# RajaeeKh/TriNerfLet

Measured on AMD Instinct MI355X. Metric: train rays/sec (whole node), higher is better.
Workload: dtype f16; 1 GPU; base: 3x32ch x 2048^2 planes, bior6.8 scale 32, hidden 64, 60000 rays/step/GPU, solid-sphere occupancy r=0.8 (re-imposed after each refresh), fp16 planes + fp16 MFMA MLP, fp32 masters, Adam+L1; GT colours = an analytic function of the ray direction (synthetic.target_colors), not a second seeded field's render; sample_budget_M=4769546, parallelism=ray-dp1

## Files before the change

### include/trinerflet_hip.h

```cpp
#ifndef TRINERFLET_HIP_H
#define TRINERFLET_HIP_H

#include <stdint.h>

#ifdef __cplusplus
extern "C" {
#endif

#define TNL_API __attribute__((visibility("default")))

TNL_API int tnl_abi_version(void);


TNL_API int tnl_near_far_from_aabb(const float *rays_o, const float *rays_d, const float *aabb,
                                   uint32_t N, float min_near, float *nears, float *fars,
                                   void *stream);

TNL_API int tnl_sph_from_ray(const float *rays_o, const float *rays_d, float radius, uint32_t N,
                             float *coords, void *stream);

TNL_API int tnl_morton3D(const int32_t *coords, uint32_t N, int32_t *indices, void *stream);

TNL_API int tnl_morton3D_invert(const int32_t *indices, uint32_t N, int32_t *coords, void *stream);

TNL_API int tnl_packbits(const float *grid, uint32_t N, float density_thresh, uint8_t *bitfield,
                         void *stream);
TNL_API int tnl_packbits_dev(const float *grid, uint32_t N, float density_thresh, const float *mean_density_dev,
                             uint8_t *bitfield, void *stream);

TNL_API int tnl_occupancy_bounds(const uint8_t *bitfield, uint32_t bytes_per_cascade, uint32_t cascades,
                                 int32_t *bounds, void *stream);
TNL_API int tnl_occupancy_row_extents(const uint8_t *bitfield, uint32_t bytes_per_cascade, uint32_t cascades, uint32_t H,
                                      float bound, uint32_t R, int32_t *ext, void *stream);

TNL_API int tnl_occupied_box(const uint8_t *bitfield, uint32_t bytes_per_cascade, uint32_t cascades, uint32_t H,
                             float bound, int32_t *bounds_scratch, float *box, void *stream);
TNL_API int tnl_clip_fars(const float *rays_o, const float *rays_d, const float *fars, const float *box, uint32_t N,
                          float *fars_out, void *stream);

TNL_API uint32_t tnl_march_rays_train_workspace(uint32_t N);
TNL_API uint32_t tnl_march_rays_train_workspace_rec(uint32_t N, uint32_t max_steps);

TNL_API int tnl_march_rays_train(const float *rays_o, const float *rays_d, const uint8_t *grid,
                                 float bound, float dt_gamma, uint32_t max_steps, uint32_t N,
                                 uint32_t C, uint32_t H, uint32_t M, const float *nears,
                                 const float *fars, float *xyzs, float *dirs, float *deltas,
                                 int32_t *rays, int32_t *counter, const float *noises,
                                 int32_t *workspace, uint32_t workspace_words, void *stream);
TNL_API int tnl_march_rays_train_binned(const float *rays_o, const float *rays_d, const uint8_t *grid,
                                 float bound, float dt_gamma, uint32_t max_steps, uint32_t N,
                                 uint32_t C, uint32_t H, uint32_t M, const float *nears,
                                 const float *fars, float *xyzs, float *dirs, float *deltas,
                                 int32_t *rays, int32_t *counter, const float *noises,
                                 int32_t *workspace, uint32_t workspace_words, uint32_t R, void *sort_workspace, void *stream);

TNL_API int tnl_march_count_form(int form);

TNL_API int tnl_march_emit_cap(int blocks);
TNL_API int tnl_plane_grad_fill_cap(int blocks);

TNL_API int tnl_composite_rays_train_forward(const float *sigmas, const float *rgbs,
                                             const float *deltas, const int32_t *rays, uint32_t M,
                                             uint32_t N, float T_thresh, float *weights_sum,
                                             float *depth, float *image, void *stream);

TNL_API int tnl_composite_rays_train_backward(const float *grad_weights_sum, const float *grad_image,
                                              const float *sigmas, const float *rgbs,
                                              const float *deltas, const int32_t *rays,
                                              const float *weights_sum, const float *image,
                                              uint32_t M, uint32_t N, float T_thresh,
                                              float *grad_sigmas, float *grad_rgbs, void *stream);

TNL_API int tnl_march_rays(uint32_t n_alive, uint32_t n_step, const int32_t *rays_alive,
                           const float *rays_t, const float *rays_o, const float *rays_d,
                           float bound, float dt_gamma, uint32_t max_steps, uint32_t C, uint32_t H,
                           const uint8_t *grid, const float *nears, const float *fars, float *xyzs,
                           float *dirs, float *deltas, const float *noises, void *stream);

TNL_API int tnl_composite_rays(uint32_t n_alive, uint32_t n_step, float T_thresh,
                               int32_t *rays_alive, float *rays_t, const float *sigmas,
                               const float *rgbs, const float *deltas, float *weights_sum,
                               float *depth, float *image, void *stream);

TNL_API int tnl_compact_rays(const int32_t *rays_alive, uint32_t n_alive, int32_t *rays_alive_out,
                             int32_t *n_out, int32_t *workspace, void *stream);

TNL_API int tnl_sh_encode_forward(const float *inputs, float *outputs, uint32_t B, uint32_t D,
                                  uint32_t C, float *dy_dx, void *stream);
TNL_API int tnl_sh_encode_backward(const float *grad, const float *inputs, uint32_t B, uint32_t D,
                                   uint32_t C, const float *dy_dx, float *grad_inputs, void *stream);


TNL_API int tnl_idwt_level_forward(const float *x, const float *yh, uint32_t S, uint32_t n,
                                   int wave, float *out, void *stream);

TNL_API int tnl_idwt_level_forward_half(const float *x, const float *yh, uint32_t S, uint32_t n,
                                        int wave, void *out_half, void *stream);

TNL_API int tnl_idwt_level_backward(const float *dout, uint32_t S, uint32_t n, int wave, float *dx,
                                    float *dyh, void *stream);

TNL_API int tnl_idwt_level_backward_adam(const float *dout, uint32_t S, uint32_t n, int wave, float *dx,
                                         float *p, float *m, float *v, float *ll_p, float *ll_m,
                                         float *ll_v, float step_size, float bias2_sqrt, float beta1,
                                         float beta2, float eps, float inv_scale,
                                         const float *inv_scale_dev, float l1_coef,
                                         const float *found_inf, float *abs_sum, void *stream);

TNL_API int tnl_planes_to_texel_major(const float *planes_cm, uint32_t C, uint32_t R, int half_out,
                                      void *planes_tm, void *stream);
TNL_API int tnl_planes_to_texel_major_win(const float *planes_cm, uint32_t C, uint32_t R, int half_out,
                                          void *planes_tm, const int32_t *roi, void *stream);
TNL_API int tnl_planes_half_to_texel_major(const void *planes_cm_half, uint32_t C, uint32_t R,
                                           void *planes_tm_half, void *stream);
TNL_API int tnl_planes_to_channel_major(const float *grad_tm, uint32_t C, uint32_t R, float *grad_cm,
                                        void *stream);

TNL_API int tnl_triplane_sample_forward(const void *planes_tm, int half_in, const float *xyz,
                                        float bound, uint32_t N, uint32_t C, uint32_t R, float *feats,
                                        void *stream);
TNL_API int tnl_triplane_sample_backward(const float *grad_feats, const float *xyz, float bound,
                                         uint32_t N, uint32_t C, uint32_t R, float *grad_tm,
                                         void *stream);

TNL_API int tnl_grid_sample_tm_forward(const void *planes_tm, int half_in, const float *grid, uint32_t N, uint32_t C,
                                       uint32_t CG, uint32_t R, float *feats, void *stream);
TNL_API int tnl_grid_sample_tm_backward(const void *planes_tm, int half_in, const float *grid,
                                        const float *grad_feats, uint32_t N, uint32_t C, uint32_t CG, uint32_t R,
                                        float *grad_tm, float *grad_grid, void *stream);

TNL_API uint32_t tnl_field_packed_bytes(uint32_t C, uint32_t Hd, uint32_t Hc);
TNL_API int tnl_field_pack(const float *W0, const float *W1, const float *W2, const float *W3,
                           const float *W4, uint32_t C, uint32_t Hd, uint32_t Hc, void *packed,
                           void *stream);
TNL_API uint64_t tnl_field_feats_save_bytes(uint32_t M, uint32_t C, uint32_t Hd);
TNL_API int tnl_field_forward(const void *planes_tm, int half_in, const float *xyz, const float *dirs,
                              float bound, uint32_t M, uint32_t C, uint32_t R, uint32_t Hd,
                              uint32_t Hc, const void *packed, float *sigma, float *rgb,
                              void *feats_save, const int32_t *m_actual, void *stream);
TNL_API uint64_t tnl_field_backward_workspace(uint32_t M, uint32_t C, uint32_t Hd, uint32_t Hc);
TNL_API int tnl_field_backward(const float *grad_sigma, const float *grad_rgb, const float *sigma,
                               const float *rgb, const void *feats_save, const float *xyz,
                               const float *dirs, float bound, uint32_t M, uint32_t C, uint32_t R,
                               uint32_t Hd, uint32_t Hc, const void *packed, float *grad_tm,
                               float *gradW, void *workspace, const int32_t *m_actual, void *dfeat_half,
                               void *stream);

TNL_API uint64_t tnl_plane_grad_binned_workspace(uint32_t M, uint32_t R);
TNL_API int tnl_plane_grad_binned(const void *dfeat_half, const float *xyz, float bound, uint32_t M,
                                  const int32_t *m_actual, uint32_t C, uint32_t R, float grad_scale,
                                  float *grad_out, int channel_major, int32_t *nonfinite_flag,
                                  void *workspace, void *stream);

TNL_API int tnl_plane_grad_sort_layout(uint32_t M, uint32_t R, int64_t *out);
TNL_API int tnl_plane_grad_sort(const float *xyz, float bound, uint32_t M, const int32_t *m_actual, uint32_t R,
                                void *workspace, void *stream);
TNL_API int tnl_plane_grad_sort_counted(const float *xyz, float bound, uint32_t M, const int32_t *m_actual,
                                        uint32_t R, void *workspace, void *stream);
TNL_API int tnl_plane_grad_reduce(const void *dfeat_half, const float *xyz, float bound, uint32_t M, uint32_t C,
                                  uint32_t R,
                                  float grad_scale, float *grad_out, int channel_major, int32_t *nonfinite_flag,
                                  const int32_t *roi, const void *workspace, void *stream);

TNL_API int tnl_idwt_level_forward_half_roi(const float *x, const float *yh, uint32_t S, uint32_t n, int wave,
                                            void *out_half, const int32_t *roi, void *stream);
TNL_API int tnl_planes_half_to_texel_major_roi(const void *planes_roi_half, uint32_t C, uint32_t R,
                                               void *planes_tm_half, const int32_t *roi, void *stream);
TNL_API int tnl_plane_grad_binned_roi(const void *dfeat_half, const float *xyz, float bound, uint32_t M,
                                      const int32_t *m_actual, uint32_t C, uint32_t R, float grad_scale,
                                      float *grad_out, int channel_major, int32_t *nonfinite_flag,
                                      const int32_t *roi, void *workspace, void *stream);
TNL_API int tnl_idwt_level_backward_roi(const float *dout_roi, uint32_t S, uint32_t n, int wave, float *dx,
                                        float *dyh, const int32_t *roi, void *stream);

TNL_API int tnl_adam_l1_step(float *p, float *grad, float *m, float *v, uint64_t n, float step_size,
                             float bias2_sqrt, float beta1, float beta2, float eps, float inv_scale,
                             const float *inv_scale_dev, float l1_coef, const float *found_inf,
                             float *abs_sum, int zero_grad, void *stream);
TNL_API int tnl_adam_l1_step_dev(float *p, float *grad, float *m, float *v, uint64_t n, float lr,
                                 const float *opt_step_dev, float beta1, float beta2, float eps, float inv_scale,
                                 const float *inv_scale_dev, float l1_coef, const float *found_inf,
                                 float *abs_sum, int zero_grad, void *stream);
TNL_API int tnl_adam_l1_step_sink(float *p, float *grad, float *m, float *v, uint64_t n, float lr,
                                  const float *opt_step_dev, float beta1, float beta2, float eps,
                                  const float *inv_scale_dev, float l1_coef, const float *l1_scaled_dev,
                                  const float *found_inf, void *stream);

TNL_API int tnl_mse_loss(const float *image, const float *weights_sum, const float *gt_rgb, float bg_color,
                         const float *bg_rays, uint32_t N, float inv_norm, const float *scale_dev, float *pred,
                         float *grad_pred, float *grad_weights_sum, float *mse_accum, void *stream);

TNL_API uint64_t tnl_abs_mean_workspace(void);
TNL_API int tnl_abs_mean_forward(const float *x, uint64_t n, void *workspace, float *out, void *stream);
TNL_API int tnl_abs_mean_backward(const float *x, uint64_t n, const float *grad_out, float *grad_x, void *stream);
TNL_API int tnl_nonfinite_check(const float *x, uint64_t n, float *found_inf, void *stream);

TNL_API int tnl_copy_probe(const void *src, void *dst, uint64_t bytes, void *stream);

TNL_API int tnl_step_prologue(const float *scale, float *inv_scale, float *abs_sum, int32_t *nonfinite, float *mse,
                              float *small_grad, uint32_t n, void *stream);
TNL_API int tnl_scaler_probe(const float *g0, uint32_t n0, const float *g1, uint32_t n1, const int32_t *nonfinite,
                             float *probe, float *found_inf, void *stream);
TNL_API int tnl_step_epilogue(const float *found_inf, float *opt_steps, float *scale, int32_t *growth_tracker,
                              float growth, float backoff, int32_t growth_interval, int32_t update_scale,
                              const float *abs_sum, float l1_coef, float *reg, void *stream);

TNL_API uint64_t tnl_permute_index(uint64_t g, uint64_t total, uint64_t key);
TNL_API int tnl_ray_batch(const float *poses, const float *intrinsics_host, uint32_t B, uint32_t H, uint32_t W,
                          const void *images, int channels, int images_u8, const int64_t *pix, uint64_t first,
                          uint64_t perm_total, uint64_t perm_key, uint32_t N, float bg_color,
                          const float *bg_rand, float *rays_o, float *rays_d, float *gt_rgb, int64_t *pix_out,
                          void *stream);

TNL_API int tnl_render_work(int units);

TNL_API int tnl_render_rays(const void *planes_tm, int half_in, uint32_t C, uint32_t R, uint32_t Hd, uint32_t Hc,
                            const void *packed, const float *rays_o, const float *rays_d, const float *nears,
                            const float *fars, uint32_t N, const uint8_t *grid, float bound, float dt_gamma,
                            uint32_t max_steps, uint32_t cascades, uint32_t H, float T_thresh, float density_scale,
                            const float *noises, int32_t *queue, float *weights_sum, float *depth, float *image,
                            void *stream);

TNL_API int tnl_infer_plan(int32_t *state, uint32_t N, uint32_t max_steps, uint32_t min_step, void *stream);
TNL_API int tnl_march_rays_dev(const int32_t *state, uint32_t N, const int32_t *rays_alive, const float *rays_t,
                               const float *rays_o, const float *rays_d, float bound, float dt_gamma,
                               uint32_t max_steps, uint32_t C, uint32_t H, const uint8_t *grid, const float *fars,
                               float *xyzs, float *dirs, float *deltas, const float *noises, float *t_scratch,
                               uint32_t rows_cap, void *stream);
TNL_API int tnl_composite_rays_dev(const int32_t *state, uint32_t N, float T_thresh, int32_t *rays_alive,
                                   float *rays_t, const float *sigmas, const float *rgbs, const float *deltas,
                                   float *weights_sum, float *depth, float *image, void *stream);
TNL_API int tnl_compact_rays_dev(int32_t *state, uint32_t N, const int32_t *rays_alive, int32_t *rays_alive_out,
                                 int32_t *workspace, void *stream);

TNL_API int tnl_idwt_level_forward_win(const float *x, const float *yh, uint32_t S, uint32_t n, int wave, float *out,
                                       const int32_t *win, void *stream);
TNL_API int tnl_idwt_level_backward_win(const float *dout, uint32_t S, uint32_t n, int wave, float *dx, float *dyh,
                                        const int32_t *win, int strided, int32_t *out_rect, void *stream);

TNL_API int tnl_idwt_set_walk_min_n(uint32_t walk_min_n);
TNL_API int tnl_idwt_get_walk_min_n(void);
TNL_API int tnl_idwt_level_forward_spans(const float *x, const float *yh, uint32_t S, uint32_t n, int wave, void *out,
                                         int half_out, const int32_t *win, int strided, const int32_t *spans,
                                         void *stream);
TNL_API int tnl_idwt_level_backward_spans(const float *dout, uint32_t S, uint32_t n, int wave, float *dx, float *dyh,
                                          const int32_t *win, int strided, int32_t *out_rect, const int32_t *spans,
                                          void *stream);
TNL_API int tnl_idwt_level_backward_live_adam(const float *dout, uint32_t S, uint32_t n, int wave, float *dx,
                                              const int32_t *win, int strided, const int32_t *live_rect,
                                              const int32_t *spans, float *p, float *m, float *v,
                                              const int32_t *band_table, uint32_t nb, const float *step_rec,
                                              float beta1, float beta2, float eps, float inv_scale,
                                              const float *inv_scale_dev, float l1_coef, const float *found_inf,
                                              float *abs_sum, void *stream);
TNL_API int tnl_planes_half_to_texel_major_spans(const void *planes_roi_half, uint32_t C, uint32_t R,
                                                 void *planes_tm_half, const int32_t *roi, const int32_t *spans,
                                                 void *stream);
TNL_API int tnl_idwt_set_tuning(int key, int value);
TNL_API int tnl_adam_l1_step_rect(float *p, float *grad, float *m, float *v, uint32_t S, uint32_t bands, uint32_t n,
                                  uint32_t spp, uint32_t s0, const int32_t *rect, float lr,
                                  const float *opt_step_dev, float beta1, float beta2, float eps, float inv_scale,
                                  const float *inv_scale_dev, float l1_coef, const float *found_inf,
                                  float *abs_sum, void *stream);
TNL_API int tnl_adam_record_step_dev(float *ring, int32_t slot, const float *lr_dev, const float *opt_step_dev, float beta1,
                                     float beta2, const float *found_inf, void *stream);
TNL_API int tnl_adam_l1_step_rec(float *p, float *grad, float *m, float *v, uint64_t n, const float *step_rec, float beta1,
                                 float beta2, float eps, const float *inv_scale_dev, float l1_coef,
                                 const float *found_inf, float *abs_sum, void *stream);
TNL_API int tnl_adam_l1_step_rect_rec(float *p, float *grad, float *m, float *v, uint32_t S, uint32_t bands, uint32_t n,
                                      uint32_t spp, uint32_t s0, const int32_t *rect, const float *step_rec, float beta1,
                                      float beta2, float eps, const float *inv_scale_dev, float l1_coef,
                                      const float *found_inf, float *abs_sum, void *stream);
TNL_API int tnl_adam_l1_step_live(float *p, float *grad, float *m, float *v, uint32_t S, uint32_t spp, uint32_t s0,
                                  uint32_t n_levels, const uint64_t *offsets, const uint32_t *sizes,
                                  const uint32_t *bands, const int32_t *live, const int32_t *grad_rect,
                                  const float *l1_coefs, float lr, const float *opt_step_dev, const float *step_rec,
                                  float beta1, float beta2, float eps, float inv_scale, const float *inv_scale_dev,
                                  const float *found_inf, float *abs_sum, void *stream);
TNL_API int tnl_adam_record_step(float *ring, int32_t slot, float lr, const float *opt_step_dev, float beta1,
                                 float beta2, const float *found_inf, void *stream);
TNL_API int tnl_adam_record_step_l1(float *ring, int32_t slot, float lr, const float *opt_step_dev, float beta1,
                                    float beta2, const float *found_inf, const float *l1_scaled_dev,
                                    const float *inv_scale_dev, void *stream);
TNL_API int tnl_adam_l1_catchup(float *p, float *m, float *v, uint32_t S, uint32_t bands, uint32_t n, uint32_t spp,
                                uint32_t s0, const int32_t *live, const float *ring, int32_t count, float beta1,
                                float beta2, float eps, float l1_coef, float *abs_sums, void *stream);
TNL_API int tnl_adam_l1_step_live_bands(float *p, float *grad, float *m, float *v, uint32_t S, uint32_t spp, uint32_t s0,
                                        uint32_t n_levels, const uint64_t *offsets, const uint32_t *sizes,
                                        const uint32_t *bands, const int32_t *live, const int32_t *grad_rect,
                                        const int32_t *const *band_tables, const uint32_t *band_quads,
                                        const float *l1_coefs, float lr, const float *opt_step_dev, const float *step_rec,
                                        float beta1, float beta2, float eps, float inv_scale, const float *inv_scale_dev,
// ... 11 lines not shown
```

### trinerflet_amd/csrc/field.hip

```cpp
#include <hip/hip_fp16.h>
#include <hip/hip_runtime.h>
#include <stdint.h>

#include "../../include/trinerflet_hip.h"
#include "field_device.h"

namespace {

#ifndef TNL_FWD_PREFETCH
#define TNL_FWD_PREFETCH 1
#endif
#ifndef TNL_FWD_LDSW
#define TNL_FWD_LDSW 0
#endif
#ifndef TNL_FWD_MINWAVES
#define TNL_FWD_MINWAVES 1
#endif
template <int C, int H, bool HALFP, bool DENSITY_ONLY, bool SAVE>
__global__ void __launch_bounds__(FWD_THREADS, TNL_FWD_MINWAVES)
k_field_fwd(const void* __restrict__ planes, const float* __restrict__ xyz, const float* __restrict__ dirs,
            float bound, uint32_t M, int R, const half8* __restrict__ packed, float* __restrict__ sigma,
            float* __restrict__ rgb, _Float16* __restrict__ feats_save, _Float16* __restrict__ geo_save,
            const int32_t* __restrict__ m_actual) {
  using G = FieldGeom<C, H>;
  if (m_actual != nullptr) M = min(M, (uint32_t)max(*m_actual, 0));
  if (M == 0) return;
  extern __shared__ __attribute__((aligned(16))) char smem[];
  half8* w = reinterpret_cast<half8*>(smem);
  constexpr int NFR = DENSITY_ONLY ? G::F2 : G::NF;
  constexpr int FT = FWD_THREADS;
  for (int i = threadIdx.x; i < NFR * 64; i += FT) w[i] = packed[i];
  __syncthreads();

  const int lane = threadIdx.x & 63, r = lane & 31, h = lane >> 5;
  const uint32_t waves = gridDim.x * (FT / 64);
  const uint32_t ntiles = (M + 31) / 32;
  const uint32_t tile0 = blockIdx.x * (FT / 64) + (threadIdx.x >> 6);
  float npx = 0.f, npy = 0.f, npz = 0.f, ndx = 0.f, ndy = 0.f, ndz = 0.f;
  auto fetch_pos = [&](uint32_t t) {
    const uint32_t i_ = t * 32 + r;
    const uint32_t il_ = i_ < M ? i_ : M - 1;
    npx = xyz[(size_t)il_ * 3]; npy = xyz[(size_t)il_ * 3 + 1]; npz = xyz[(size_t)il_ * 3 + 2];
    if (!DENSITY_ONLY) { ndx = dirs[(size_t)il_ * 3]; ndy = dirs[(size_t)il_ * 3 + 1]; ndz = dirs[(size_t)il_ * 3 + 2]; }
  };
  if (tile0 < ntiles) fetch_pos(tile0);
  for (uint32_t tile = tile0; tile < ntiles; tile += waves) {
#if TNL_FWD_LDSW
    asm volatile("" : "+s"(w));
#endif
    const uint32_t i = tile * 32 + r;
    const bool valid = i < M;
    const float px = npx, py = npy, pz = npz;
    const float cdx = ndx, cdy = ndy, cdz = ndz;
    if (tile + waves < ntiles) fetch_pos(tile + waves);
#ifndef TNL_FWD_PG128
#define TNL_FWD_PG128 1
#endif
    constexpr int PG = H > 64 ? TNL_FWD_PG128 : 3;
    const uint32_t il = valid ? i : M - 1;
    f32x16 acc0[G::OB];
#pragma unroll
    for (int ob = 0; ob < G::OB; ob++) acc0[ob] = zero16();
#pragma unroll
    for (int p0 = 0; p0 < 3; p0 += PG) {
      half8 fk[PG * (C / 16)];
#pragma unroll
      for (int p = p0; p < p0 + PG; p++) {
        TexelTap t;
        triplane_tap(px, py, pz, bound, R, p, t);
#pragma unroll
        for (int kk = 0; kk < C / 16; kk++) fk[(p - p0) * (C / 16) + kk] = gather_frag<C, HALFP>(planes, R, p, kk, h, t);
      }
      if (TNL_FWD_PREFETCH && H > 64) {
#pragma unroll
        for (int q = 0; q < PG * (C / 16); q++)
          if (SAVE) *reinterpret_cast<half8*>(feats_save + feat_slot<G::KS0>(il, p0 * (C / 16) + q, h)) = fk[q];
        with_weights<PG * (C / 16) * G::OB, G::OB>(
            [&](int i) { return w[(G::F0 + (i % G::OB) * G::KS0 + p0 * (C / 16) + i / G::OB) * 64 + lane]; },
            [&](int i, const half8& f) { acc0[i % G::OB] = MFMA32(f, fk[i / G::OB], acc0[i % G::OB]); });
      } else {
#pragma unroll
        for (int q = 0; q < PG * (C / 16); q++) {
          const int ks = p0 * (C / 16) + q;
          if (SAVE) *reinterpret_cast<half8*>(feats_save + feat_slot<G::KS0>(il, ks, h)) = fk[q];
#pragma unroll
          for (int ob = 0; ob < G::OB; ob++) acc0[ob] = MFMA32(w[(G::F0 + ob * G::KS0 + ks) * 64 + lane], fk[q], acc0[ob]);
        }
      }
      if (PG < 3) __builtin_amdgcn_sched_barrier(0);
    }
    const float dx = cdx, dy = cdy, dz = cdz;
    Chain<C, H> ch;
    chain_tail<C, H, DENSITY_ONLY, (TNL_FWD_PREFETCH && H > 64)>(w, w, lane, h, acc0, dx, dy, dz, ch);
    if (!DENSITY_ONLY && geo_save != nullptr && valid) {
      half8 g;
#pragma unroll
      for (int j = 0; j < 8; j++) g[j] = (_Float16)ch.o8[j];
      *reinterpret_cast<half8*>(geo_save + (size_t)i * 16 + 8 * h) = g;
    }
    if (valid && h == 0) {
      sigma[i] = expf(ch.o8[0]);
      if (!DENSITY_ONLY) {
        rgb[(size_t)i * 3 + 0] = 1.f / (1.f + expf(-ch.rgbl[0]));
        rgb[(size_t)i * 3 + 1] = 1.f / (1.f + expf(-ch.rgbl[1]));
        rgb[(size_t)i * 3 + 2] = 1.f / (1.f + expf(-ch.rgbl[2]));
      }
    }
    if (DENSITY_ONLY && rgb != nullptr && valid) {
#pragma unroll
      for (int g = 0; g < 8; g++) {
        const int row = acc_row(g, h);
        if (row >= 1) rgb[(size_t)i * 15 + row - 1] = ch.o8[g];
      }
    }
  }
}

template <int C, int H>
__global__ void k_field_pack(const float* __restrict__ W0, const float* __restrict__ W1, const float* __restrict__ W2,
                             const float* __restrict__ W3, const float* __restrict__ W4,
                             _Float16* __restrict__ packed) {
  using G = FieldGeom<C, H>;
  const int idx = blockIdx.x * blockDim.x + threadIdx.x;
  if (idx >= G::NTOT * 512) return;
  const int src = field_pack_source<C, H>(idx);
  float v = 0.f;
  if (src >= 0) {
    if (src < G::OFF1) v = W0[src - G::OFF0];
    else if (src < G::OFF2) v = W1[src - G::OFF1];
    else if (src < G::OFF3) v = W2[src - G::OFF2];
    else if (src < G::OFF4) v = W3[src - G::OFF3];
    else v = W4[src - G::OFF4];
  }
  packed[idx] = (_Float16)v;
}

template <int C, int H>
int launch_fwd(const void* planes, int half_in, const float* xyz, const float* dirs, float bound, uint32_t M,
               uint32_t R, const void* packed, float* sigma, float* rgb, void* feats_save, bool density_only,
               const int32_t* m_actual, hipStream_t st) {
  using G = FieldGeom<C, H>;
  const uint32_t ntiles = (M + 31) / 32;
  constexpr uint32_t WPB = FWD_THREADS / 64;
  uint32_t blocks = (ntiles + WPB - 1) / WPB;
  if (blocks > 2048) blocks = 2048;
  const half8* pk = reinterpret_cast<const half8*>(packed);
  _Float16* fs = reinterpret_cast<_Float16*>(feats_save);
  _Float16* gs = (split_backward<H>() && fs != nullptr) ? fs + (size_t)((M + 31) / 32 * 32) * G::F : nullptr;
#define TNL_LAUNCH(HP, DO, SV)                                                                                        \
  hipLaunchKernelGGL((k_field_fwd<C, H, HP, DO, SV>), dim3(blocks), dim3(FWD_THREADS), (DO ? G::F2 : G::NF) * 1024, st, \
                     planes, xyz, dirs, bound, M, (int)R, pk, sigma, rgb, fs, gs, m_actual)
#define TNL_LAUNCH_SV(HP, DO) do { if (fs != nullptr) TNL_LAUNCH(HP, DO, true); else TNL_LAUNCH(HP, DO, false); } while (0)
  if (density_only) {
    if (half_in) TNL_LAUNCH_SV(true, true); else TNL_LAUNCH_SV(false, true);
  } else {
    if (half_in) TNL_LAUNCH_SV(true, false); else TNL_LAUNCH_SV(false, false);
  }
#undef TNL_LAUNCH_SV
#undef TNL_LAUNCH
  return (int)hipGetLastError();
}

}

int tnl_field_forward_h128(const void* planes, int half_in, const float* xyz, const float* dirs, float bound, uint32_t M,
                           uint32_t R, const void* packed, float* sigma, float* rgb, void* feats_save, bool density_only,
                           const int32_t* m_actual, hipStream_t st);
#ifdef TNL_FIELD_H128_ONLY
int tnl_field_forward_h128(const void* planes, int half_in, const float* xyz, const float* dirs, float bound, uint32_t M,
                           uint32_t R, const void* packed, float* sigma, float* rgb, void* feats_save, bool density_only,
                           const int32_t* m_actual, hipStream_t st) {
  return launch_fwd<48, 128>(planes, half_in, xyz, dirs, bound, M, R, packed, sigma, rgb, feats_save, density_only, m_actual, st);
}
#else

extern "C" {

uint32_t tnl_field_packed_bytes(uint32_t C, uint32_t Hd, uint32_t Hc) {
  if (Hd != Hc) return 0;
  if (C == 16 && Hd == 64) return FieldGeom<16, 64>::NTOT * 1024;
  if (C == 32 && Hd == 64) return FieldGeom<32, 64>::NTOT * 1024;
  if (C == 48 && Hd == 128) return FieldGeom<48, 128>::NTOT * 1024;
  return 0;
}

uint64_t tnl_field_feats_save_bytes(uint32_t M, uint32_t C, uint32_t Hd) {
  return ((uint64_t)((M + 31) / 32) * 32 * 3 * C + (uint64_t)M * (Hd > 64 ? 16 : 0)) * 2;
}

int tnl_field_pack(const float* W0, const float* W1, const float* W2, const float* W3, const float* W4, uint32_t C,
                   uint32_t Hd, uint32_t Hc, void* packed, void* stream) {
  if (Hd != Hc) return (int)hipErrorInvalidValue;
  hipStream_t st = (hipStream_t)stream;
  _Float16* pk = reinterpret_cast<_Float16*>(packed);
#define TNL_PACK(CC, HH)                                                                                      \
  hipLaunchKernelGGL((k_field_pack<CC, HH>), dim3((FieldGeom<CC, HH>::NTOT * 512 + 255) / 256), dim3(256), 0, st, \
                     W0, W1, W2, W3, W4, pk)
  if (C == 16 && Hd == 64) TNL_PACK(16, 64);
  else if (C == 32 && Hd == 64) TNL_PACK(32, 64);
  else if (C == 48 && Hd == 128) TNL_PACK(48, 128);
  else return (int)hipErrorInvalidValue;
#undef TNL_PACK
  return (int)hipGetLastError();
}

int tnl_field_forward(const void* planes_tm, int half_in, const float* xyz, const float* dirs, float bound,
                      uint32_t M, uint32_t C, uint32_t R, uint32_t Hd, uint32_t Hc, const void* packed,
                      float* sigma, float* rgb, void* feats_save, const int32_t* m_actual, void* stream) {
  if (M == 0) return 0;
  if (Hd != Hc) return (int)hipErrorInvalidValue;
  hipStream_t st = (hipStream_t)stream;
  const bool density_only = (dirs == nullptr) || (rgb == nullptr);
  if (C == 16 && Hd == 64)
    return launch_fwd<16, 64>(planes_tm, half_in, xyz, dirs, bound, M, R, packed, sigma, rgb, feats_save, density_only, m_actual, st);
  if (C == 32 && Hd == 64)
    return launch_fwd<32, 64>(planes_tm, half_in, xyz, dirs, bound, M, R, packed, sigma, rgb, feats_save, density_only, m_actual, st);
  if (C == 48 && Hd == 128)
    return tnl_field_forward_h128(planes_tm, half_in, xyz, dirs, bound, M, R, packed, sigma, rgb, feats_save, density_only, m_actual, st);
  return (int)hipErrorInvalidValue;
}

}
#endif
```

### trinerflet_amd/csrc/field_device.h

```cpp
#pragma once
#include <hip/hip_fp16.h>
#include <hip/hip_runtime.h>
#include <stdint.h>

#include "field_common.h"
#include "triplane_common.h"

namespace {

#define MFMA32(a, b, c) __builtin_amdgcn_mfma_f32_32x32x16_f16((a), (b), (c), 0, 0, 0)

constexpr int FWD_THREADS = 256;

template <typename K>
inline hipError_t ensure_dynamic_lds(K kernel, int bytes, bool (&done)[64]) {
  int dev = 0;
  (void)hipGetDevice(&dev);
  if (dev >= 0 && dev < 64 && done[dev]) return hipSuccess;
  const hipError_t e = hipFuncSetAttribute(reinterpret_cast<const void*>(kernel), hipFuncAttributeMaxDynamicSharedMemorySize, bytes);
  if (e == hipSuccess && dev >= 0 && dev < 64) done[dev] = true;
  return e;
}

__device__ __forceinline__ f32x16 zero16() {
  f32x16 z;
#pragma unroll
  for (int i = 0; i < 16; i++) z[i] = 0.f;
  return z;
}

template <bool RELU>
__device__ __forceinline__ half8 acc_to_frag(const f32x16& a, int s) {
  half8 f;
#pragma unroll
  for (int j = 0; j < 8; j++) f[j] = (_Float16)(s == 0 ? a[j] : a[8 + j]);
  if (RELU) {
    const half8 z = {0, 0, 0, 0, 0, 0, 0, 0};
    f = __builtin_elementwise_max(f, z);
  }
  return f;
}

__device__ __forceinline__ half8 relu_mask_frag(half8 d, half8 x) {
  typedef uint32_t u32x4 __attribute__((ext_vector_type(4)));
  u32x4 db = __builtin_bit_cast(u32x4, d);
  const u32x4 xb = __builtin_bit_cast(u32x4, x);
#pragma unroll
  for (int q = 0; q < 4; q++) {
    uint32_t t, m;
    asm("v_pk_add_u16 %0, %1, %2" : "=v"(t) : "v"(xb[q]), "s"(0x7fff7fffu));
    asm("v_pk_ashrrev_i16 %0, %1, %2" : "=v"(m) : "s"(0x000f000fu), "v"(t));
    db[q] &= m;
  }
  return __builtin_bit_cast(half8, db);
}

__device__ __forceinline__ half8 sh_frag(float x, float y, float z, int h) {
  const float xy = x * y, xz = x * z, yz = y * z, x2 = x * x, y2 = y * y, z2 = z * z;
  half8 f;
  if (h == 0) {
    f[0] = (_Float16)0.28209479177387814f;
    f[1] = (_Float16)(-0.48860251190291987f * y);
    f[2] = (_Float16)(0.48860251190291987f * z);
    f[3] = (_Float16)(-0.48860251190291987f * x);
    f[4] = (_Float16)(1.0925484305920792f * xy);
    f[5] = (_Float16)(-1.0925484305920792f * yz);
    f[6] = (_Float16)(0.94617469575755997f * z2 - 0.31539156525251999f);
    f[7] = (_Float16)(-1.0925484305920792f * xz);
  } else {
    f[0] = (_Float16)(0.54627421529603959f * x2 - 0.54627421529603959f * y2);
    f[1] = (_Float16)(0.59004358992664352f * y * (-3.0f * x2 + y2));
    f[2] = (_Float16)(2.8906114426405538f * xy * z);
    f[3] = (_Float16)(0.45704579946446572f * y * (1.0f - 5.0f * z2));
    f[4] = (_Float16)(0.3731763325901154f * z * (5.0f * z2 - 3.0f));
    f[5] = (_Float16)(0.45704579946446572f * x * (1.0f - 5.0f * z2));
    f[6] = (_Float16)(1.4453057213202769f * z * (x2 - y2));
    f[7] = (_Float16)(0.59004358992664352f * x * (-x2 + 3.0f * y2));
  }
  return f;
}

template <bool HALFP>
__device__ __forceinline__ void load8(const void* planes, size_t elem, float (&v)[8]) {
  if (HALFP) {
    const half8 t = *reinterpret_cast<const half8*>(reinterpret_cast<const _Float16*>(planes) + elem);
#pragma unroll
    for (int j = 0; j < 8; j++) v[j] = (float)t[j];
  } else {
    const float4* p = reinterpret_cast<const float4*>(reinterpret_cast<const float*>(planes) + elem);
    const float4 a = p[0], b = p[1];
    v[0] = a.x; v[1] = a.y; v[2] = a.z; v[3] = a.w; v[4] = b.x; v[5] = b.y; v[6] = b.z; v[7] = b.w;
  }
}

template <int C, bool HALFP>
__device__ __forceinline__ half8 gather_frag(const void* planes, int R, int p, int kk, int h, const TexelTap& t) {
  const int c0 = 16 * kk + 8 * h;
  const size_t pb = (size_t)p * R * R;
  float v00[8], v01[8], v10[8], v11[8];
  load8<HALFP>(planes, (pb + (size_t)t.y0 * R + t.x0) * C + c0, v00);
  load8<HALFP>(planes, (pb + (size_t)t.y0 * R + t.x1) * C + c0, v01);
  load8<HALFP>(planes, (pb + (size_t)t.y1 * R + t.x0) * C + c0, v10);
  load8<HALFP>(planes, (pb + (size_t)t.y1 * R + t.x1) * C + c0, v11);
  half8 f;
#pragma unroll
  for (int j = 0; j < 8; j++)
    f[j] = (_Float16)(v00[j] * t.w00 + v01[j] * t.w01 + v10[j] * t.w10 + v11[j] * t.w11);
  return f;
}

template <int N, int GROUP, class WSrc, class Body>
__device__ __forceinline__ void with_weights(WSrc wsrc, Body body) {
  constexpr int NG = (N + GROUP - 1) / GROUP;
  half8 buf[2][GROUP];
#pragma unroll
  for (int j = 0; j < GROUP; j++)
    if (j < N) buf[0][j] = wsrc(j);
#pragma unroll
  for (int g = 0; g < NG; g++) {
#pragma unroll
    for (int j = 0; j < GROUP; j++)
      if (g + 1 < NG && (g + 1) * GROUP + j < N) buf[(g + 1) & 1][j] = wsrc((g + 1) * GROUP + j);
#pragma unroll
    for (int j = 0; j < GROUP; j++)
      if (g * GROUP + j < N) body(g * GROUP + j, buf[g & 1][j]);
    __builtin_amdgcn_sched_barrier(0);
  }
}

template <int C, int H>
struct Chain {
  using G = FieldGeom<C, H>;
  half8 h1[G::KH];
  float o8[8];
  half8 h3[G::KH];
  half8 h4[G::KH];
  float rgbl[3];
};

template <int C, int H>
__device__ __forceinline__ const half8& wfrag(const half8* w, int f, int lane) { return w[f * 64 + lane]; }

template <int C, int H, bool FENCE = false>
__device__ __forceinline__ void chain_colour(const half8* w, const half8* wH, int lane, int h, const half8 geo,
                                             float dx, float dy, float dz, Chain<C, H>& ch);

template <int C, int H, bool DENSITY_ONLY, bool FENCE = false>
__device__ __forceinline__ void chain_tail(const half8* w, const half8* wH, int lane, int h, f32x16 (&acc0)[H / 32],
                                           float dx, float dy, float dz, Chain<C, H>& ch) {
  using G = FieldGeom<C, H>;
#pragma unroll
  for (int ks = 0; ks < G::KH; ks++) {
    ch.h1[ks] = (ks & 1) ? acc_to_frag<true>(acc0[ks >> 1], 1) : acc_to_frag<true>(acc0[ks >> 1], 0);
  }
  f32x16 o = zero16();
  if (FENCE) {
    with_weights<G::KH, 4>([&](int i) { return w[(G::F1 + i) * 64 + lane]; },
                           [&](int i, const half8& f) { o = MFMA32(f, ch.h1[i], o); });
  } else {
#pragma unroll
    for (int ks = 0; ks < G::KH; ks++) o = MFMA32(w[(G::F1 + ks) * 64 + lane], ch.h1[ks], o);
  }
#pragma unroll
  for (int g = 0; g < 8; g++) ch.o8[g] = o[g];
  if (DENSITY_ONLY) return;
  chain_colour<C, H, FENCE>(w, wH, lane, h, acc_to_frag<false>(o, 0), dx, dy, dz, ch);
}

template <int C, int H, bool FENCE>
__device__ __forceinline__ void chain_colour(const half8* w, const half8* wH, int lane, int h, const half8 geo,
                                             float dx, float dy, float dz, Chain<C, H>& ch) {
  using G = FieldGeom<C, H>;
  const half8 shf = sh_frag(dx, dy, dz, h);
  f32x16 acc2[G::OB];
#pragma unroll
  for (int ob = 0; ob < G::OB; ob++) {
    acc2[ob] = MFMA32(w[(G::F2 + 2 * ob) * 64 + lane], shf, zero16());
    acc2[ob] = MFMA32(w[(G::F2 + 2 * ob + 1) * 64 + lane], geo, acc2[ob]);
  }
#pragma unroll
  for (int ks = 0; ks < G::KH; ks++)
    ch.h3[ks] = (ks & 1) ? acc_to_frag<true>(acc2[ks >> 1], 1) : acc_to_frag<true>(acc2[ks >> 1], 0);
  f32x16 out = zero16();
  if (FENCE) {
    f32x16 t3a = zero16(), t3b = zero16();
    auto post3 = [&](int ob, const f32x16& t) { ch.h4[2 * ob] = acc_to_frag<true>(t, 0); ch.h4[2 * ob + 1] = acc_to_frag<true>(t, 1); };
    with_weights<G::OB * G::KH, 4>([&](int i) { return wH[(G::F3 + i) * 64 + lane]; }, [&](int i, const half8& f) {
      const int ob = i / G::KH, ks = i % G::KH;
      f32x16& t3 = (ob & 1) ? t3b : t3a;
      if (ks == 0) t3 = zero16();
      t3 = MFMA32(f, ch.h3[ks], t3);
      if (ks == 3 && ob > 0) post3(ob - 1, (ob & 1) ? t3a : t3b);
      if (i == G::OB * G::KH - 1) post3(ob, t3);
    });
    with_weights<G::KH, 4>([&](int i) { return wH[(G::F4 + i) * 64 + lane]; },
                           [&](int i, const half8& f) { out = MFMA32(f, ch.h4[i], out); });
  } else {
    f32x16 acc3[G::OB];
#pragma unroll
    for (int ob = 0; ob < G::OB; ob++) {
      acc3[ob] = zero16();
#pragma unroll
      for (int ks = 0; ks < G::KH; ks++) acc3[ob] = MFMA32(wH[(G::F3 + ob * G::KH + ks) * 64 + lane], ch.h3[ks], acc3[ob]);
    }
#pragma unroll
    for (int ks = 0; ks < G::KH; ks++)
      ch.h4[ks] = (ks & 1) ? acc_to_frag<true>(acc3[ks >> 1], 1) : acc_to_frag<true>(acc3[ks >> 1], 0);
#pragma unroll
    for (int ks = 0; ks < G::KH; ks++) out = MFMA32(wH[(G::F4 + ks) * 64 + lane], ch.h4[ks], out);
  }
  ch.rgbl[0] = out[0]; ch.rgbl[1] = out[1]; ch.rgbl[2] = out[2];
}


}
```

### trinerflet_amd/nerf/field.py

```python
import ctypes as C

import torch
from torch.autograd import Function

from .. import _lib as L

SUPPORTED = {(16, 64), (32, 64), (48, 128)}


def supported(C, Hd, Hc):
    return Hd == Hc and (C, Hd) in SUPPORTED


def pack_weights(W0, W1, W2, W3, W4, C, H):
    lib = L.lib()
    nbytes = lib.tnl_field_packed_bytes(L.u32(C), L.u32(H), L.u32(H))
    if nbytes == 0:
        raise NotImplementedError(f"fused field: unsupported (channels={C}, hidden={H})")
    packed = torch.empty(nbytes // 2, dtype=torch.float16, device=W0.device)
    ws = [w.detach().to(torch.float32).contiguous() for w in (W0, W1, W2, W3, W4)]
    L.check(lib.tnl_field_pack(*[L.ptr(w) for w in ws], L.u32(C), L.u32(H), L.u32(H), L.ptr(packed), L.stream()),
            "field_pack")
    return packed


def field_forward(planes_tm, xyz, dirs, packed, bound, C, R, H, save_feats=False, geo_out=False, m_actual=None,
                  zero_tail=False):
    M = xyz.shape[0]
    dev = xyz.device
    new = torch.zeros if (zero_tail and m_actual is not None) else torch.empty
    sigma = new(M, dtype=torch.float32, device=dev)
    if dirs is None:
        second = new(M, 15, dtype=torch.float32, device=dev) if geo_out else None
    else:
        second = new(M, 3, dtype=torch.float32, device=dev)
    feats = None
    if save_feats:
        nb = L.lib().tnl_field_feats_save_bytes(L.u32(M), L.u32(C), L.u32(H))
        feats = torch.empty(nb // 2, dtype=torch.float16, device=dev)
    L.check(L.lib().tnl_field_forward(L.ptr(planes_tm), L.i32(int(planes_tm.dtype == torch.float16)), L.ptr(xyz),
                                      L.ptr(dirs), L.f32(bound), L.u32(M), L.u32(C), L.u32(R), L.u32(H), L.u32(H),
                                      L.ptr(packed), L.ptr(sigma), L.ptr(second), L.ptr(feats), L.ptr(m_actual), L.stream()),
            "field_forward")
    return sigma, second, feats


def field_backward(grad_sigma, grad_rgb, sigma, rgb, feats, xyz, dirs, packed, bound, C, R, H, grad_tm, gradW,
                   m_actual=None, dfeat=None):
    lib = L.lib()
    M = xyz.shape[0]
    nws = lib.tnl_field_backward_workspace(L.u32(M), L.u32(C), L.u32(H), L.u32(H))
    ws = torch.empty(max(nws, 4), dtype=torch.uint8, device=xyz.device)
    L.check(lib.tnl_field_backward(L.ptr(grad_sigma), L.ptr(grad_rgb), L.ptr(sigma), L.ptr(rgb), L.ptr(feats),
                                   L.ptr(xyz), L.ptr(dirs), L.f32(bound), L.u32(M), L.u32(C), L.u32(R), L.u32(H),
                                   L.u32(H), L.ptr(packed), L.ptr(grad_tm), L.ptr(gradW), L.ptr(ws), L.ptr(m_actual), L.ptr(dfeat),
                                   L.stream()),
            "field_backward")


_SIDE = {}


def _side_stream(device):
    key = (device.type, device.index if device.index is not None else torch.cuda.current_device())
    if key not in _SIDE:
        _SIDE[key] = torch.cuda.Stream(device=device)
    return _SIDE[key]


class _FusedField(Function):
    binned_backward = True
    early_sort = True
    deterministic = False

    @staticmethod
    def forward(ctx, planes_tm, xyz, dirs, W0, W1, W2, W3, W4, bound, planes_cm=None, m_actual=None, window=None):
        L.require_cuda(planes_tm, xyz, dirs, W0)
        _, R, _, C = planes_tm.shape
        H = W0.shape[0]
        xyz = xyz.detach().to(torch.float32).contiguous()
        dirs = dirs.detach().to(torch.float32).contiguous()
        packed = pack_weights(W0, W1, W2, W3, W4, C, H)
        need_grad = any(ctx.needs_input_grad)
        if m_actual is not None:
            m_actual = m_actual.reshape(-1)[:1].to(torch.int32).clone()
        ctx.m_actual = m_actual
        ctx.window = [int(v) for v in window] if (window is not None and planes_cm is not None) else None
        ctx.sort = None
        if (need_grad and _FusedField.early_sort and R % 32 == 0 and _FusedField.binned_backward and xyz.shape[0] > 0
                and ctx.needs_input_grad[0 if planes_cm is None else 9]):
            cur = torch.cuda.current_stream()
            side = _side_stream(xyz.device)
            side.wait_stream(cur)
            with torch.cuda.stream(side):
                ws = plane_grad_sort(xyz, float(bound), R, m_actual)
                if _FusedField.deterministic:
                    order_tile_lists(ws, R, xyz.shape[0])
                ev = torch.cuda.Event()
                ev.record()
            ws.record_stream(cur)
            for t_ in (xyz,) + ((m_actual,) if m_actual is not None else ()):
                t_.record_stream(side)
            ctx.sort = (ws, ev)
        sigma, rgb, feats = field_forward(planes_tm, xyz, dirs, packed, float(bound), C, R, H, save_feats=need_grad,
                                          m_actual=m_actual, zero_tail=True)
        ctx.save_for_backward(xyz, dirs, packed, sigma, rgb, feats)
        ctx.dims = (C, R, H, float(bound), [tuple(w.shape) for w in (W0, W1, W2, W3, W4)])
        ctx.cm = planes_cm is not None and R % 32 == 0 and _FusedField.binned_backward
        if planes_cm is not None and not ctx.cm:
            raise NotImplementedError("fused_field(planes_cm=...) needs plane_resolution % 32 == 0 (the tile reduction)")
        return sigma, rgb

    @staticmethod
    def backward(ctx, g_sigma, g_rgb):
        xyz, dirs, packed, sigma, rgb, feats = ctx.saved_tensors
        C, R, H, bound, shapes = ctx.dims
        dev = xyz.device
        g_sigma = g_sigma.to(torch.float32).contiguous()
        g_rgb = g_rgb.to(torch.float32).contiguous()
        nw = sum(a * b for a, b in shapes)
        gradW = torch.zeros(nw, dtype=torch.float32, device=dev)
        if ctx.cm:
            win = ctx.window if xyz.shape[0] > 0 else None
            grad_cm = (torch.empty if win is not None else torch.zeros)(3, C, R, R, dtype=torch.float32, device=dev)
            if xyz.shape[0] > 0:
                dfeat = torch.empty(3, xyz.shape[0], C, dtype=torch.float16, device=dev)
                field_backward(g_sigma, g_rgb, sigma, rgb, feats, xyz, dirs, packed, bound, C, R, H, grad_cm, gradW, dfeat=dfeat,
                               m_actual=ctx.m_actual)
                kw = dict(roi=win + [C, 0], roi_in_place=True) if win is not None else dict(prezeroed=True)
                if ctx.sort is not None:
                    torch.cuda.current_stream().wait_event(ctx.sort[1])
                    plane_grad_reduce(ctx.sort[0], dfeat, xyz, bound, C, R, grad_cm, channel_major=True, **kw)
                elif _FusedField.deterministic:
                    ws = plane_grad_sort(xyz, bound, R, ctx.m_actual)
                    order_tile_lists(ws, R, xyz.shape[0])
                    plane_grad_reduce(ws, dfeat, xyz, bound, C, R, grad_cm, channel_major=True, **kw)
                else:
                    plane_grad_binned(dfeat, xyz, bound, C, R, grad_cm, m_actual=ctx.m_actual, channel_major=True, **kw)
            grad_tm = None
        elif R % 32 == 0 and xyz.shape[0] > 0 and _FusedField.binned_backward:
            grad_tm = torch.zeros(3, R, R, C, dtype=torch.float32, device=dev)
            dfeat = torch.empty(3, xyz.shape[0], C, dtype=torch.float16, device=dev)
            field_backward(g_sigma, g_rgb, sigma, rgb, feats, xyz, dirs, packed, bound, C, R, H, grad_tm, gradW, dfeat=dfeat,
                           m_actual=ctx.m_actual)
            if ctx.sort is not None:
                torch.cuda.current_stream().wait_event(ctx.sort[1])
                plane_grad_reduce(ctx.sort[0], dfeat, xyz, bound, C, R, grad_tm, prezeroed=True)
            elif _FusedField.deterministic:
                ws = plane_grad_sort(xyz, bound, R, ctx.m_actual)
                order_tile_lists(ws, R, xyz.shape[0])
                plane_grad_reduce(ws, dfeat, xyz, bound, C, R, grad_tm, prezeroed=True)
            else:
                plane_grad_binned(dfeat, xyz, bound, C, R, grad_tm, m_actual=ctx.m_actual, prezeroed=True)
        else:
            grad_tm = torch.zeros(3, R, R, C, dtype=torch.float32, device=dev)
            field_backward(g_sigma, g_rgb, sigma, rgb, feats, xyz, dirs, packed, bound, C, R, H, grad_tm, gradW,
                           m_actual=ctx.m_actual)
        gws, off = [], 0
        for a, b in shapes:
            gws.append(gradW[off:off + a * b].view(a, b))
            off += a * b
        return (grad_tm, None, None, *gws, None, grad_cm if ctx.cm else None, None, None)


fused_field = _FusedField.apply


def plane_grad_sort(xyz, bound, R, m_actual=None):
    lib = L.lib()
    M = xyz.shape[0]
    nbytes = lib.tnl_plane_grad_binned_workspace(L.u32(M), L.u32(R))
    if nbytes == 0:
        raise NotImplementedError("binned plane gradient needs plane_resolution % 32 == 0")
    ws = torch.empty(nbytes, dtype=torch.uint8, device=xyz.device)
    L.check(lib.tnl_plane_grad_sort(L.ptr(xyz), L.f32(bound), L.u32(M), L.ptr(m_actual), L.u32(R), L.ptr(ws),
                                    L.stream()), "plane_grad_sort")
# ... 68 lines not shown
```

Before: 15.52 million rays/s.

## Stage triplane texel gathers through LDS via global_load_lds in fused field forward

Adds an alternative forward gather path for hidden-64 fields. Each wave issues global_load_lds direct-to-LDS loads of the four bilinear corner texels per plane, using shuffled texel addresses and a rotated layout to spread LDS banks. Lanes then read their fragments from LDS and blend them, instead of issuing per-lane 16-byte global gathers. The path is chosen automatically when the extra LDS fits the device limit, with a thread-local override and a Python context manager. It costs extra LDS per block, which may lower occupancy, and adds explicit waitcnt serialization between planes.

```diff
diff --git a/include/trinerflet_hip.h b/include/trinerflet_hip.h
--- a/include/trinerflet_hip.h
+++ b/include/trinerflet_hip.h
@@ -138,6 +138,8 @@
                               float bound, uint32_t M, uint32_t C, uint32_t R, uint32_t Hd,
                               uint32_t Hc, const void *packed, float *sigma, float *rgb,
                               void *feats_save, const int32_t *m_actual, void *stream);
+TNL_API int tnl_field_fwd_gather_form(int form);
+TNL_API int tnl_field_fwd_gather_form_of(uint32_t C, uint32_t Hd, int half_in, uint32_t lds_limit_bytes);
 TNL_API uint64_t tnl_field_backward_workspace(uint32_t M, uint32_t C, uint32_t Hd, uint32_t Hc);
 TNL_API int tnl_field_backward(const float *grad_sigma, const float *grad_rgb, const float *sigma,
                                const float *rgb, const void *feats_save, const float *xyz,
diff --git a/trinerflet_amd/csrc/field.hip b/trinerflet_amd/csrc/field.hip
--- a/trinerflet_amd/csrc/field.hip
+++ b/trinerflet_amd/csrc/field.hip
@@ -16,7 +16,12 @@
 #ifndef TNL_FWD_MINWAVES
 #define TNL_FWD_MINWAVES 1
 #endif
-template <int C, int H, bool HALFP, bool DENSITY_ONLY, bool SAVE>
+template <int C, int H, bool HALFP>
+constexpr int fwd_lds_bytes(bool density_only, bool ldsg) {
+  return ((density_only ? FieldGeom<C, H>::F2 : FieldGeom<C, H>::NF) + (ldsg ? 4 * GatherLds<C, HALFP>::NP : 0)) * 1024;
+}
+
+template <int C, int H, bool HALFP, bool DENSITY_ONLY, bool SAVE, bool LDSG = false>
 __global__ void __launch_bounds__(FWD_THREADS, TNL_FWD_MINWAVES)
 k_field_fwd(const void* __restrict__ planes, const float* __restrict__ xyz, const float* __restrict__ dirs,
             float bound, uint32_t M, int R, const half8* __restrict__ packed, float* __restrict__ sigma,
@@ -61,33 +66,56 @@
     f32x16 acc0[G::OB];
 #pragma unroll
     for (int ob = 0; ob < G::OB; ob++) acc0[ob] = zero16();
-#pragma unroll
-    for (int p0 = 0; p0 < 3; p0 += PG) {
-      half8 fk[PG * (C / 16)];
-#pragma unroll
-      for (int p = p0; p < p0 + PG; p++) {
-        TexelTap t;
-        triplane_tap(px, py, pz, bound, R, p, t);
-#pragma unroll
-        for (int kk = 0; kk < C / 16; kk++) fk[(p - p0) * (C / 16) + kk] = gather_frag<C, HALFP>(planes, R, p, kk, h, t);
-      }
-      if (TNL_FWD_PREFETCH && H > 64) {
-#pragma unroll
-        for (int q = 0; q < PG * (C / 16); q++)
-          if (SAVE) *reinterpret_cast<half8*>(feats_save + feat_slot<G::KS0>(il, p0 * (C / 16) + q, h)) = fk[q];
-        with_weights<PG * (C / 16) * G::OB, G::OB>(
-            [&](int i) { return w[(G::F0 + (i % G::OB) * G::KS0 + p0 * (C / 16) + i / G::OB) * 64 + lane]; },
-            [&](int i, const half8& f) { acc0[i % G::OB] = MFMA32(f, fk[i / G::OB], acc0[i % G::OB]); });
-      } else {
-#pragma unroll
-        for (int q = 0; q < PG * (C / 16); q++) {
-          const int ks = p0 * (C / 16) + q;
-          if (SAVE) *reinterpret_cast<half8*>(feats_save + feat_slot<G::KS0>(il, ks, h)) = fk[q];
-#pragma unroll
-          for (int ob = 0; ob < G::OB; ob++) acc0[ob] = MFMA32(w[(G::F0 + ob * G::KS0 + ks) * 64 + lane], fk[q], acc0[ob]);
+    if constexpr (LDSG) {
+      using GL = GatherLds<C, HALFP>;
+      char* const img = smem + NFR * 1024 + (threadIdx.x >> 6) * GL::PLANE_BYTES;
+      TexelTap t[3];
+#pragma unroll
+      for (int p = 0; p < 3; p++) triplane_tap(px, py, pz, bound, R, p, t[p]);
+      half8 fk[3 * (C / 16)];
+#pragma unroll
+      for (int p = 0; p < 3; p++) {
+        __builtin_amdgcn_s_waitcnt(0xc07f);
+        GL::issue(planes, R, p, t[p], lane, img);
+        __builtin_amdgcn_s_waitcnt(0x0f70);
+#pragma unroll
+        for (int kk = 0; kk < C / 16; kk++) fk[p * (C / 16) + kk] = GL::frag(img, r, h, kk, t[p]);
+      }
+#pragma unroll
+      for (int ks = 0; ks < 3 * (C / 16); ks++) {
+        if (SAVE) *reinterpret_cast<half8*>(feats_save + feat_slot<G::KS0>(il, ks, h)) = fk[ks];
+#pragma unroll
+        for (int ob = 0; ob < G::OB; ob++) acc0[ob] = MFMA32(w[(G::F0 + ob * G::KS0 + ks) * 64 + lane], fk[ks], acc0[ob]);
+      }
+    } else {
+#pragma unroll
+      for (int p0 = 0; p0 < 3; p0 += PG) {
+        half8 fk[PG * (C / 16)];
+#pragma unroll
+        for (int p = p0; p < p0 + PG; p++) {
+          TexelTap t;
+          triplane_tap(px, py, pz, bound, R, p, t);
+#pragma unroll
+          for (int kk = 0; kk < C / 16; kk++) fk[(p - p0) * (C / 16) + kk] = gather_frag<C, HALFP>(planes, R, p, kk, h, t);
         }
-      }
-      if (PG < 3) __builtin_amdgcn_sched_barrier(0);
+        if (TNL_FWD_PREFETCH && H > 64) {
+#pragma unroll
+          for (int q = 0; q < PG * (C / 16); q++)
+            if (SAVE) *reinterpret_cast<half8*>(feats_save + feat_slot<G::KS0>(il, p0 * (C / 16) + q, h)) = fk[q];
+          with_weights<PG * (C / 16) * G::OB, G::OB>(
+              [&](int i) { return w[(G::F0 + (i % G::OB) * G::KS0 + p0 * (C / 16) + i / G::OB) * 64 + lane]; },
+              [&](int i, const half8& f) { acc0[i % G::OB] = MFMA32(f, fk[i / G::OB], acc0[i % G::OB]); });
+        } else {
+#pragma unroll
+          for (int q = 0; q < PG * (C / 16); q++) {
+            const int ks = p0 * (C / 16) + q;
+            if (SAVE) *reinterpret_cast<half8*>(feats_save + feat_slot<G::KS0>(il, ks, h)) = fk[q];
+#pragma unroll
+            for (int ob = 0; ob < G::OB; ob++) acc0[ob] = MFMA32(w[(G::F0 + ob * G::KS0 + ks) * 64 + lane], fk[q], acc0[ob]);
+          }
+        }
+        if (PG < 3) __builtin_amdgcn_sched_barrier(0);
+      }
     }
     const float dx = cdx, dy = cdy, dz = cdz;
     Chain<C, H> ch;
@@ -135,10 +163,27 @@
   packed[idx] = (_Float16)v;
 }
 
+template <int C, int H, bool HP, bool DO, bool SV, class... Args>
+void launch_fwd_form(bool lds_form, uint32_t blocks, hipStream_t st, Args... args) {
+  if constexpr (H == 64 && GatherLds<C, HP>::APPLIES) {
+    if (lds_form) {
+      static bool attr_set[64] = {};
+      constexpr int lds = fwd_lds_bytes<C, H, HP>(DO, true);
+      if (ensure_dynamic_lds(&k_field_fwd<C, H, HP, DO, SV, true>, lds, attr_set) == hipSuccess) {
+        hipLaunchKernelGGL((k_field_fwd<C, H, HP, DO, SV, true>), dim3(blocks), dim3(FWD_THREADS), lds, st, args...);
+        return;
+      }
+      (void)hipGetLastError();
+    }
+  }
+  constexpr int lds = fwd_lds_bytes<C, H, HP>(DO, false);
+  hipLaunchKernelGGL((k_field_fwd<C, H, HP, DO, SV, false>), dim3(blocks), dim3(FWD_THREADS), lds, st, args...);
+}
+
 template <int C, int H>
 int launch_fwd(const void* planes, int half_in, const float* xyz, const float* dirs, float bound, uint32_t M,
                uint32_t R, const void* packed, float* sigma, float* rgb, void* feats_save, bool density_only,
-               const int32_t* m_actual, hipStream_t st) {
+               const int32_t* m_actual, bool lds_form, hipStream_t st) {
   using G = FieldGeom<C, H>;
   const uint32_t ntiles = (M + 31) / 32;
   constexpr uint32_t WPB = FWD_THREADS / 64;
@@ -147,9 +192,8 @@
   const half8* pk = reinterpret_cast<const half8*>(packed);
   _Float16* fs = reinterpret_cast<_Float16*>(feats_save);
   _Float16* gs = (split_backward<H>() && fs != nullptr) ? fs + (size_t)((M + 31) / 32 * 32) * G::F : nullptr;
-#define TNL_LAUNCH(HP, DO, SV)                                                                                        \
-  hipLaunchKernelGGL((k_field_fwd<C, H, HP, DO, SV>), dim3(blocks), dim3(FWD_THREADS), (DO ? G::F2 : G::NF) * 1024, st, \
-                     planes, xyz, dirs, bound, M, (int)R, pk, sigma, rgb, fs, gs, m_actual)
+#define TNL_LAUNCH(HP, DO, SV) \
+  launch_fwd_form<C, H, HP, DO, SV>(lds_form, blocks, st, planes, xyz, dirs, bound, M, (int)R, pk, sigma, rgb, fs, gs, m_actual)
 #define TNL_LAUNCH_SV(HP, DO) do { if (fs != nullptr) TNL_LAUNCH(HP, DO, true); else TNL_LAUNCH(HP, DO, false); } while (0)
   if (density_only) {
     if (half_in) TNL_LAUNCH_SV(true, true); else TNL_LAUNCH_SV(false, true);
@@ -170,11 +214,46 @@
 int tnl_field_forward_h128(const void* planes, int half_in, const float* xyz, const float* dirs, float bound, uint32_t M,
                            uint32_t R, const void* packed, float* sigma, float* rgb, void* feats_save, bool density_only,
                            const int32_t* m_actual, hipStream_t st) {
-  return launch_fwd<48, 128>(planes, half_in, xyz, dirs, bound, M, R, packed, sigma, rgb, feats_save, density_only, m_actual, st);
+  return launch_fwd<48, 128>(planes, half_in, xyz, dirs, bound, M, R, packed, sigma, rgb, feats_save, density_only, m_actual, false, st);
 }
 #else
 
+static thread_local int g_gather_form = 0;
+
+static uint32_t device_lds_limit() {
+  static int cached[64] = {};
+  int dev = 0, v = 0;
+  if (hipGetDevice(&dev) != hipSuccess) { (void)hipGetLastError(); return 0; }
+  if (dev >= 0 && dev < 64 && cached[dev] > 0) return (uint32_t)cached[dev];
+  if (hipDeviceGetAttribute(&v, hipDeviceAttributeMaxSharedMemoryPerBlock, dev) != hipSuccess) { (void)hipGetLastError(); return 0; }
+  if (dev >= 0 && dev < 64) cached[dev] = v;
+  return v > 0 ? (uint32_t)v : 0;
+}
+
+template <int C, int H>
+static int gather_form_of(int half_in, uint32_t lds_limit) {
+  if (g_gather_form == 1 || H != 64) return 1;
+  const bool applies = half_in ? GatherLds<C, true>::APPLIES : GatherLds<C, false>::APPLIES;
+  if (!applies) return 1;
+  const uint32_t need = half_in ? fwd_lds_bytes<C, H, true>(false, true) : fwd_lds_bytes<C, H, false>(false, true);
+  return need <= lds_limit ? 2 : 1;
+}
+
 extern "C" {
+
+int tnl_field_fwd_gather_form(int form) {
+  const int prev = g_gather_form;
+  if (form == 0 || form == 1) g_gather_form = form;
+  return prev;
+}
+
+int tnl_field_fwd_gather_form_of(uint32_t C, uint32_t Hd, int half_in, uint32_t lds_limit_bytes) {
+  const uint32_t limit = lds_limit_bytes != 0 ? lds_limit_bytes : device_lds_limit();
+  if (C == 16 && Hd == 64) return gather_form_of<16, 64>(half_in, limit);
+  if (C == 32 && Hd == 64) return gather_form_of<32, 64>(half_in, limit);
+  if (C == 48 && Hd == 128) return gather_form_of<48, 128>(half_in, limit);
+  return -1;
+}
 
 uint32_t tnl_field_packed_bytes(uint32_t C, uint32_t Hd, uint32_t Hc) {
   if (Hd != Hc) return 0;
@@ -212,9 +291,11 @@
   hipStream_t st = (hipStream_t)stream;
   const bool density_only = (dirs == nullptr) || (rgb == nullptr);
   if (C == 16 && Hd == 64)
-    return launch_fwd<16, 64>(planes_tm, half_in, xyz, dirs, bound, M, R, packed, sigma, rgb, feats_save, density_only, m_actual, st);
+    return launch_fwd<16, 64>(planes_tm, half_in, xyz, dirs, bound, M, R, packed, sigma, rgb, feats_save, density_only, m_actual,
+                              gather_form_of<16, 64>(half_in, device_lds_limit()) == 2, st);
   if (C == 32 && Hd == 64)
-    return launch_fwd<32, 64>(planes_tm, half_in, xyz, dirs, bound, M, R, packed, sigma, rgb, feats_save, density_only, m_actual, st);
+    return launch_fwd<32, 64>(planes_tm, half_in, xyz, dirs, bound, M, R, packed, sigma, rgb, feats_save, density_only, m_actual,
+                              gather_form_of<32, 64>(half_in, device_lds_limit()) == 2, st);
   if (C == 48 && Hd == 128)
     return tnl_field_forward_h128(planes_tm, half_in, xyz, dirs, bound, M, R, packed, sigma, rgb, feats_save, density_only, m_actual, st);
   return (int)hipErrorInvalidValue;
diff --git a/trinerflet_amd/csrc/field_device.h b/trinerflet_amd/csrc/field_device.h
--- a/trinerflet_amd/csrc/field_device.h
+++ b/trinerflet_amd/csrc/field_device.h
@@ -93,6 +93,15 @@
   }
 }
 
+__device__ __forceinline__ half8 blend_frag(const float (&v00)[8], const float (&v01)[8], const float (&v10)[8],
+                                            const float (&v11)[8], const TexelTap& t) {
+  half8 f;
+#pragma unroll
+  for (int j = 0; j < 8; j++)
+    f[j] = (_Float16)(v00[j] * t.w00 + v01[j] * t.w01 + v10[j] * t.w10 + v11[j] * t.w11);
+  return f;
+}
+
 template <int C, bool HALFP>
 __device__ __forceinline__ half8 gather_frag(const void* planes, int R, int p, int kk, int h, const TexelTap& t) {
   const int c0 = 16 * kk + 8 * h;
@@ -102,12 +111,60 @@
   load8<HALFP>(planes, (pb + (size_t)t.y0 * R + t.x1) * C + c0, v01);
   load8<HALFP>(planes, (pb + (size_t)t.y1 * R + t.x0) * C + c0, v10);
   load8<HALFP>(planes, (pb + (size_t)t.y1 * R + t.x1) * C + c0, v11);
-  half8 f;
-#pragma unroll
-  for (int j = 0; j < 8; j++)
-    f[j] = (_Float16)(v00[j] * t.w00 + v01[j] * t.w01 + v10[j] * t.w10 + v11[j] * t.w11);
-  return f;
-}
+  return blend_frag(v00, v01, v10, v11, t);
+}
+
+template <int C, bool HALFP>
+struct GatherLds {
+  static constexpr int E = HALFP ? 2 : 4;
+  static constexpr int NP = 2 * C * E / 16;
+  static constexpr bool APPLIES = (NP & (NP - 1)) == 0 && NP >= 4 && NP <= 16;
+  static constexpr int SPI = 64 / NP;
+  static constexpr int PLANE_BYTES = NP * 1024;
+  __device__ static __forceinline__ int rot(int rs) { return ((rs & 15) * NP) >> 4; }
+
+  __device__ static __forceinline__ void issue(const void* planes, int R, int p, const TexelTap& t, int lane, char* img) {
+    const int h = lane >> 5;
+    const uint32_t pb = (uint32_t)p * R * R, x = (uint32_t)(t.x0 + h * (t.x1 - t.x0));
+    const uint32_t texel[2] = {pb + (uint32_t)t.y0 * R + x, pb + (uint32_t)t.y1 * R + x};
+    const char* base = reinterpret_cast<const char*>(planes);
+#pragma unroll
+    for (int grp = 0; grp < NP / 2; grp++) {
+      const int rs = grp * SPI + lane / NP;
+      const int k = ((lane % NP) - rot(rs)) & (NP - 1), xb = k / (NP / 2), j = k % (NP / 2);
+#pragma unroll
+      for (int row = 0; row < 2; row++) {
+        const size_t o = (size_t)__shfl(texel[row], rs + 32 * xb) * (C * E) + 16 * j;
+        __builtin_amdgcn_global_load_lds((const __attribute__((address_space(1))) void*)(base + o),
+                                         (__attribute__((address_space(3))) void*)(img + (2 * grp + row) * 1024), 16, 0, 0);
+      }
+    }
+  }
+
+  __device__ static __forceinline__ void read8(const char* img, int r, int h, int kk, int row, int xb, float (&v)[8]) {
+    const int j = (32 * kk + 16 * h) * E / 32;
+    const char* seg = img + (2 * (r / SPI) + row) * 1024 + (r % SPI) * NP * 16;
+    const int k = xb * (NP / 2) + j + rot(r);
+    if (HALFP) {
+      const half8 a = *reinterpret_cast<const half8*>(seg + (k & (NP - 1)) * 16);
+#pragma unroll
+      for (int q = 0; q < 8; q++) v[q] = (float)a[q];
+    } else {
+      const float4 a = *reinterpret_cast<const float4*>(seg + (k & (NP - 1)) * 16);
+      const float4 b = *reinterpret_cast<const float4*>(seg + ((k + 1) & (NP - 1)) * 16);
+      v[0] = a.x; v[1] = a.y; v[2] = a.z; v[3] = a.w; v[4] = b.x; v[5] = b.y; v[6] = b.z; v[7] = b.w;
+    }
+  }
+
+  __device__ static __forceinline__ half8 frag(const char* img, int r, int h, int kk, const TexelTap& t) {
+    float v00[8], v01[8], v10[8], v11[8];
+    read8(img, r, h, kk, 0, 0, v00);
+    read8(img, r, h, kk, 0, 1, v01);
+    read8(img, r, h, kk, 1, 0, v10);
+    read8(img, r, h, kk, 1, 1, v11);
+    return blend_frag(v00, v01, v10, v11, t);
+  }
+};
 
 template <int N, int GROUP, class WSrc, class Body>
 __device__ __forceinline__ void with_weights(WSrc wsrc, Body body) {
diff --git a/trinerflet_amd/nerf/field.py b/trinerflet_amd/nerf/field.py
--- a/trinerflet_amd/nerf/field.py
+++ b/trinerflet_amd/nerf/field.py
@@ -22,6 +22,23 @@
     L.check(lib.tnl_field_pack(*[L.ptr(w) for w in ws], L.u32(C), L.u32(H), L.u32(H), L.ptr(packed), L.stream()),
             "field_pack")
     return packed
+
+
+class gather_form:
+
+    def __init__(self, form):
+        self.form = int(form)
+
+    def __enter__(self):
+        self.prev = L.lib().tnl_field_fwd_gather_form(L.i32(self.form))
+        return self
+
+    def __exit__(self, *exc):
+        L.lib().tnl_field_fwd_gather_form(L.i32(self.prev))
+
+
+def gather_form_of(C, H, half_planes, lds_limit_bytes=0):
+    return L.lib().tnl_field_fwd_gather_form_of(L.u32(C), L.u32(H), L.i32(int(bool(half_planes))), L.u32(lds_limit_bytes))
 
 
 def field_forward(planes_tm, xyz, dirs, packed, bound, C, R, H, save_feats=False, geo_out=False, m_actual=None,
```

Result: no change. 15.80 million rays/s (median of 6 runs) (+1.8%).
